# Theseus-AT/mlx-vector-db

Hardware: AMD Instinct MI355X
Metric: QPS + p50 latency, cosine top-10 batch=64: 1M×768D @1 GPU; 10M×128D @8 GPU (higher is better)
Workload: dtype f32 (int8 centred corpus x int8 query integer-MFMA candidates, fp64 exact rerank); 1 GPU; c2: 1M x 768 fp32 cosine top-10, batch 64; n_rows=1000000, dim=768, global_batch=64, batch_per_gpu_equiv=64, k=10, metric=cosine, parallelism=single GPU, rows_per_gpu=1000000

## Files before the change

### mlx-vector-db_amd/csrc/vdb_api.cpp

```cpp
#include <hip/hip_runtime.h>

#include <algorithm>
#include <atomic>
#include <cmath>
#include <cstdarg>
#include <cstdio>
#include <cstring>
#include <mutex>
#include <set>
#include <unordered_map>
#include <shared_mutex>
#include <string>
#include <vector>

#include "../../include/vdb.h"
#include "vdb_compact_plan.h"
#include "vdb_internal.h"

using namespace vdb;

namespace {

thread_local std::string g_last_error;

// ... 79 lines not shown
    float* d_dir = nullptr;
    bool dir_set = false;
    double xres_dir = 0.0;
    float* d_mu = nullptr;
    float sx = 0.0f;
    int64_t dir_rows = 0;
    unsigned long long* d_i8 = nullptr;
    double i8st[6] = {0, 0, 0, 0, 0, 0};
    uint32_t* d_csum = nullptr;
    int64_t scan_checksum = 1;
    bool auto_i8 = true;
    hipStream_t stream = nullptr;
    int n_cu = 256;
    int64_t precision = VDB_PREC_AUTO;
    std::atomic<int> auto_hold{0}, auto_fails{0}, auto_ok{0};
    std::atomic<int> auto_hold8{0}, auto_fails8{0}, auto_ok8{0};
    std::atomic<bool> last_i8{false};
    std::atomic<unsigned long long> auto_seen{0};
    unsigned long long* h_totals = nullptr;
    int64_t margin = -1;
    int64_t force_exact = 0;
    int64_t n_wg_override = 0;
    int64_t timing = 0;
    int64_t pilot_tiles = -1;
    int64_t graph_fill = 0;
    int64_t scan_variant = 0;
    int64_t scan_variant_b3 = 0;
    int64_t scan_sync = 0;
    int64_t no_fallback = 0;
    int64_t pilot_rank_override = 0;
    bool no_dir_bound = false;
    int64_t finish_split = 1;
    int64_t finish_small = -1;
    int64_t scan_qlds = -1;
    int i8_refine = -1;
    int64_t device_repass = -1;
    std::atomic<int> repass_arm{0};
    int64_t i8_narrow = -1;
    std::atomic<bool> i8_wide{false};
    std::atomic<bool> auto_i8q{true};
    std::atomic<bool> i8q_off{false};
    std::atomic<bool> last_i8q{false};
    std::atomic<int> last_i8q_b{0};
    int64_t scan_q4 = -1;
    int64_t scan_wide = -1;
    int64_t remove_chunk = 0;
    std::atomic<int64_t> gen{0};
    std::atomic<int64_t> n_searches{0}, n_queries{0}, n_fallback{0}, n_overflow{0}, n_incons{0}, n_repass{0}, n_q4{0};
    std::atomic<int64_t> n_wide{0};
    std::atomic<int64_t> n_xs_builds{0};
    std::atomic<int64_t> n_rows_removed{0};
    std::atomic<int64_t> n_by_prec[N_PREC] = {{0}, {0}, {0}, {0}, {0}, {0}};
    std::atomic<int64_t> scan_ns{0}, pipe_ns{0}, n_timed{0};
    unsigned long long* d_totals = nullptr;
    std::shared_mutex mu;
    std::mutex xs_mu;
    std::mutex ws_mu;
    std::vector<Workspace*> pool;
    std::unordered_map<hipStream_t, hipEvent_t> uses;
};

namespace {

std::mutex g_reg_mu;
std::set<vdb_index*> g_indices;

void free_workspace_memory(Workspace* w) {
    if (w->dev) (void)hipFree(w->dev);
    if (w->exact) (void)hipFree(w->exact);
    if (w->host_flag) (void)hipHostFree(w->host_flag);
    if (w->host_io) (void)hipHostFree(w->host_io);
    w->dev = nullptr;
    w->exact = nullptr;
    w->host_flag = nullptr;
    w->host_io = nullptr;
    w->dev_bytes = w->exact_bytes = w->host_io_bytes = 0;
}

int wait_idle(vdb_index* ix);

enum XsKind { kXsNone = -1, kXsFp32 = 0, kXsSplit = 1 };
int xs_kind(int64_t precision) {
// ... 536 lines not shown
        }
        if (xq && ix->X && ix->count > 0) {
            HIP_TRY(build_candidate_rows(ix, 0, ix->count, ix->stream, false, true));
            HIP_TRY(read_i8_stats(ix, ix->stream));
        }
    } else if (n == "margin") {
        ix->margin = value;
    } else if (n == "force_exact") {
        ix->force_exact = value != 0;
    } else if (n == "n_wg") {
        ix->n_wg_override = value;
    } else if (n == "scan_sync") {
        if (value < 0 || value > 2) return set_error(VDB_ERR_INVALID, "scan_sync must be 0, 1 or 2");
        ix->scan_sync = value;
    } else if (n == "scan_variant") {
        if (value < 0 || value > 2) return set_error(VDB_ERR_INVALID, "scan_variant must be 0, 1 or 2");
        ix->scan_variant = value;
    } else if (n == "scan_variant_bf16x3") {
        if (value != 0) return set_error(VDB_ERR_INVALID, "the split-bf16 pass has one variant (0)");
        ix->scan_variant_b3 = value;
    } else if (n == "graph_fill") {
        if (value < 0 || value > 1) return set_error(VDB_ERR_INVALID, "graph_fill must be 0 or 1");
        ix->graph_fill = value;
    } else if (n == "pilot_tiles") {
        if (value < -1 || value > 32768) return set_error(VDB_ERR_INVALID, "pilot_tiles must be in [-1, 32768]");
        ix->pilot_tiles = value;
    } else if (n == "timing") {
        ix->timing = value != 0;
    } else if (n == "no_fallback") {
        ix->no_fallback = value != 0;
    } else if (n == "finish_small") {
        if (value < -1 || value > 1) return set_error(VDB_ERR_INVALID, "finish_small must be -1, 0 or 1");
        ix->finish_small = value;
    } else if (n == "finish_split") {
        if (value < 1 || value > 8) return set_error(VDB_ERR_INVALID, "finish_split must be in [1, 8]");
        ix->finish_split = value;
    } else if (n == "scan_qlds") {
        if (value < -1 || value > 2) return set_error(VDB_ERR_INVALID, "scan_qlds must be -1 (auto), 0, 1 or 2");
        ix->scan_qlds = value;
    } else if (n == "scan_wide") {
        if (value < -1 || value > 1) return set_error(VDB_ERR_INVALID, "scan_wide must be -1, 0 or 1");
        ix->scan_wide = value;
    } else if (n == "scan_q4") {
        if (value < -1 || value > 1) return set_error(VDB_ERR_INVALID, "scan_q4 must be -1, 0 or 1");
        ix->scan_q4 = value;
    } else if (n == "dir_bound") {
        ix->no_dir_bound = value == 0;
    } else if (n == "i8_refine") {
        if (value < -1 || value > 1) return set_error(VDB_ERR_INVALID, "i8_refine must be -1, 0 or 1");
        ix->i8_refine = (int)value;
    } else if (n == "i8_narrow") {
        if (value < -1 || value > 0) return set_error(VDB_ERR_INVALID, "i8_narrow must be -1 or 0");
        ix->i8_narrow = value;
    } else if (n == "remove_chunk") {
        if (value < 0) return set_error(VDB_ERR_INVALID, "remove_chunk must be >= 0 (0 = sized by bytes)");
        std::unique_lock<std::shared_mutex> g(ix->mu);
        ix->remove_chunk = value;
    } else if (n == "device_repass") {
        if (value < -1 || value > 1) return set_error(VDB_ERR_INVALID, "device_repass must be -1, 0 or 1");
        ix->device_repass = value;
    } else if (n.rfind("debug_", 0) == 0 && !debug_knobs_enabled()) {
        return set_error(VDB_ERR_INVALID, "'%s' is a test-only knob (set VDB_DEBUG_KNOBS=1)", name);
    } else if (n == "debug_sink_row8") {
        HIP_TRY(hipSetDevice(ix->device));
        std::unique_lock<std::shared_mutex> g(ix->mu);
        if (value < 0 || value >= ix->count || !ix->Xq)
// ... 16 lines not shown
        HIP_TRY(hipMemcpyAsync(ix->rinit32 + value, &zero, sizeof(float), hipMemcpyHostToDevice, ix->stream));
        HIP_TRY(hipStreamSynchronize(ix->stream));
    } else if (n == "pilot_rank") {
        if (value < 0 || value > 256) return set_error(VDB_ERR_INVALID, "pilot_rank must be in [0, 256]");
        ix->pilot_rank_override = value;
    } else {
        return set_error(VDB_ERR_INVALID, "unknown parameter '%s'", name);
    }
    return VDB_OK;
}

int32_t vdb_index_get_stat(const vdb_index* cix, const char* name, int64_t* value) {
    if (!cix || !name || !value) return set_error(VDB_ERR_INVALID, "NULL argument");
    vdb_index* ix = const_cast<vdb_index*>(cix);
    std::string n(name);
    unsigned long long dt[4] = {0, 0, 0, 0};
    if ((n == "fallback_queries" || n == "overflow_queries" || n == "repass_queries") && ix->d_totals) {
        HIP_TRY(hipSetDevice(ix->device));
        const int wr = wait_idle(ix);
        if (wr) return wr;
        HIP_TRY(hipMemcpy(dt, ix->d_totals, sizeof(dt), hipMemcpyDeviceToHost));
    }
    if (n == "scan_ns" || n == "pipeline_ns" || n == "timed_searches") {
        HIP_TRY(hipSetDevice(ix->device));
        const int rc = flush_all_timing(ix);
        if (rc) return rc;
    }
    if (n == "searches") *value = ix->n_searches.load();
    else if (n == "queries") *value = ix->n_queries.load();
    else if (n == "fallback_queries") *value = ix->n_fallback.load() + (int64_t)dt[0];
    else if (n == "repass_queries") *value = ix->n_repass.load() + (int64_t)dt[3];
    else if (n == "searches_q4") *value = ix->n_q4.load();
    else if (n == "searches_wide") *value = ix->n_wide.load();
    else if (n == "auto_hold") *value = ix->auto_hold.load();
    else if (n == "auto_hold8") *value = ix->auto_hold8.load();
    else if (n == "overflow_queries") *value = ix->n_overflow.load() + (int64_t)dt[1];
    else if (n == "inconsistent_queries") *value = ix->n_incons.load();
    else if (n == "capacity") *value = ix->cap_rows;
    else if (n == "scan_ns") *value = ix->scan_ns.load();
    else if (n == "pipeline_ns") *value = ix->pipe_ns.load();
    else if (n == "timed_searches") *value = ix->n_timed.load();
    else if (n == "count") *value = ix->count;
    else if (n == "precision") *value = ix->precision;
    else if (n == "searches_fp32") *value = ix->n_by_prec[PREC_FP32].load();
    else if (n == "searches_bf16x3") *value = ix->n_by_prec[PREC_BF16X3].load();
    else if (n == "searches_bf16") *value = ix->n_by_prec[PREC_BF16].load();
    else if (n == "searches_i8") *value = ix->n_by_prec[PREC_I8].load();
    else if (n == "searches_i8x3") *value = ix->n_by_prec[PREC_I8X3].load();
    else if (n == "auto_int8") *value = ix->auto_i8 ? 1 : 0;
    else if (n == "auto_i8q") *value = ix->auto_i8q ? 1 : 0;
    else if (n == "i8q_off") *value = ix->i8q_off.load() ? 1 : 0;
    else if (n == "searches_i8q") *value = ix->n_by_prec[PREC_I8Q].load();
    else if (n == "i8_wide") *value = ix->i8_wide ? 1 : 0;
    else if (n == "device_bytes") {
        const int64_t xb = (int64_t)(ix->cap_rows / 32) * ix->G * BLOCK_FLOATS * 4;
        *value = xb + (xs_ptr(ix) ? xb : 0) + (ix->Xq ? xb / 2 : 0) + (ix->Xh ? xb / 4 : 0) + ix->cap_rows * 20;
    } else if (n == "split_copy") *value = xs_ptr(ix) ? 1 : 0;
    else if (n == "split_copy_builds") *value = ix->n_xs_builds.load();
    else if (n == "rows_removed") *value = ix->n_rows_removed.load();
    else return set_error(VDB_ERR_INVALID, "unknown stat '%s'", name);
    return VDB_OK;
}

constexpr int64_t kDirRows = 65536;

static hipError_t setup_direction(vdb_index* ix, int64_t row0, int64_t n, hipStream_t st) {
// ... 325 lines not shown
    if (!ix || (!out_host && n > 0)) return set_error(VDB_ERR_INVALID, "NULL argument");
    if (start < 0 || n < 0 || start + n > ix->count)
        return set_error(VDB_ERR_INVALID, "rows [%lld, %lld) out of range [0, %lld)", (long long)start,
                         (long long)(start + n), (long long)ix->count);
    if (n == 0) return VDB_OK;
    HIP_TRY(hipSetDevice(ix->device));
    std::shared_lock<std::shared_mutex> g(ix->mu);
    const int D = ix->dim;
    const int64_t chunk = std::max<int64_t>(1, (int64_t)(256ll << 20) / ((int64_t)D * 4));
    float* tmp = nullptr;
    HIP_TRY(hipMalloc(&tmp, (size_t)std::min(chunk, n) * D * sizeof(float)));
    for (int64_t r = 0; r < n; r += chunk) {
        const int64_t m = std::min(chunk, n - r);
        hipError_t e = launch_unpack_rows(ix->X, ix->G, D, start + r, m, tmp, ix->stream);
        if (e == hipSuccess)
            e = hipMemcpyAsync(out_host + r * D, tmp, (size_t)m * D * sizeof(float), hipMemcpyDeviceToHost, ix->stream);
        if (e == hipSuccess) e = hipStreamSynchronize(ix->stream);
        if (e != hipSuccess) {
            (void)hipFree(tmp);
            return set_error(VDB_ERR_HIP, "export failed: %s", hipGetErrorString(e));
        }
    }
    (void)hipFree(tmp);
    return VDB_OK;
}

constexpr int32_t kRetryBf16x3 = 1 << 20;
constexpr int kRepassMax = 64;
constexpr int kRepassDev = 16;
constexpr int kRepassArm = 256;
constexpr int64_t kI8NarrowRows = 512 * 1024;
constexpr int64_t kI8NarrowRowsShort = 4 * 1024 * 1024;
constexpr int64_t kWideMinRows = 65536;
constexpr int64_t kWideSplitMaxRows = 2500000;
constexpr int FIN_SEG_MAX = 512;
constexpr int64_t kRefineMinDp = 512;
constexpr int kAutoBf16MaxK = 16;

void auto_fail(vdb_index* ix) {
    const int f = std::min(8, ix->auto_fails.load() + 1);
    ix->auto_fails = f;
    ix->auto_ok = 0;
    ix->auto_hold = 16 << (f - 1);
}

bool auto_take_hold(vdb_index* ix) {
    int h = ix->auto_hold.load();
    while (h > 0)
        if (ix->auto_hold.compare_exchange_weak(h, h - 1)) return true;
    if (++ix->auto_ok >= 64) ix->auto_fails = 0;
    return false;
}

void auto_fail8(vdb_index* ix) {
    const int f = std::min(8, ix->auto_fails8.load() + 1);
    ix->auto_fails8 = f;
    ix->auto_ok8 = 0;
    ix->auto_hold8 = 16 << (f - 1);
}
bool auto_take_hold8(vdb_index* ix) {
    int h = ix->auto_hold8.load();
    while (h > 0)
        if (ix->auto_hold8.compare_exchange_weak(h, h - 1)) return true;
    if (++ix->auto_ok8 >= 64) ix->auto_fails8 = 0;
    return false;
}
// ... 242 lines not shown
    Carver c{w->dev};
    float* Qraw = c.take<float>((size_t)B * D);
    uint32_t* maskd = c.take<uint32_t>(mask_words + 64);
    float* Qt = c.take<float>((size_t)Bp * (ix->Dp + 16 * QG_EXTRA));
    double* qn64 = c.take<double>(Bp);
    double* qconst = c.take<double>((size_t)Bp * 3);
    const float* q_mu = i8_pass ? ix->d_mu : nullptr;
    const float* q_dir = (prec == PREC_BF16 || i8_pass) && ix->dir_set && !ix->no_dir_bound ? ix->d_dir : nullptr;
    float* os = c.take<float>((size_t)B * k);
    int64_t* oi = c.take<int64_t>((size_t)B * k);
    double* ok = c.take<double>((size_t)B * k);
    int* flags = c.take<int>(B + 64);
    int* done = c.take<int>(Bp);
    uint32_t* gthr = c.take<uint32_t>(Bp);
    uint32_t* gslots = c.take<uint32_t>((size_t)Bp * (KP_MAX + PILOT_SLOTS));
    uint32_t* pslots = gslots + (size_t)Bp * KP_MAX;
    float* gl_s = c.take<float>((size_t)B * gl_cap);
    uint32_t* gl_i = c.take<uint32_t>((size_t)B * gl_cap);
    uint32_t* gl_cnt = c.take<uint32_t>(Bp);
    double* fx_ek = fin_split > 1 ? c.take<double>((size_t)B * fin_split * KP_MAX) : nullptr;
    uint32_t* fx_ck = fin_split > 1 ? c.take<uint32_t>((size_t)B * fin_split * KP_MAX) : nullptr;
    uint32_t* fx_cr = fin_split > 1 ? c.take<uint32_t>((size_t)B * fin_split * KP_MAX) : nullptr;
    int* fx_n = fin_split > 1 ? c.take<int>((size_t)B * fin_split) : nullptr;
    float* q8max = c.take<float>(Bp);
    float* q8lsl = c.take<float>(Bp);
    float* q8err = c.take<float>(Bp);
    float* q8scal = c.take<float>(64);
    float* q8res = i8_refine ? c.take<float>((size_t)Bp * ix->Dp) : nullptr;
    float* q8err2 = i8_refine ? c.take<float>(Bp) : nullptr;
    uint32_t* chkp = chk ? c.take<uint32_t>((size_t)2 * n_wg8 * Bp) : nullptr;
    uint32_t* segc = wide8 ? c.take<uint32_t>((size_t)Bp * n_seg8) : nullptr;
    uint32_t* chkr = chk && ix->metric == 1 ? c.take<uint32_t>(64) : nullptr;
    int* rs8 = rs8_on ? c.take<int>((size_t)round_up(N, 32)) : nullptr;
    uint32_t* chke = chk && n_pilot > 0 ? c.take<uint32_t>((size_t)2 * Bp) : nullptr;
    float* rep_q = mem == VDB_MEM_DEVICE ? c.take<float>((size_t)R_rep * D) : nullptr;
    float* rep_s = mem == VDB_MEM_DEVICE ? c.take<float>((size_t)R_rep * k) : nullptr;
    int64_t* rep_i = mem == VDB_MEM_DEVICE ? c.take<int64_t>((size_t)R_rep * k) : nullptr;
    double* rep_k = mem == VDB_MEM_DEVICE ? c.take<double>((size_t)R_rep * k) : nullptr;

    const float* Qd = queries;
    const uint32_t* md = row_mask;
    float* out_s = out_scores;
    int64_t* out_i = out_indices;
    double* out_k = out_keys;
    const size_t io_q = mem == VDB_MEM_HOST ? (size_t)B * D * 4 : 0;
    const size_t io_r = (size_t)B * k * (4 + 8 + (out_keys ? 8 : 0));
    bool staged = false;
    if (mem == VDB_MEM_HOST) {
        rc = ws_host_io(w, io_q + io_r);
        if (rc) return rc;
        std::memcpy(w->host_io, queries, io_q);
        HIP_TRY(hipMemcpyAsync(Qraw, w->host_io, io_q, hipMemcpyHostToDevice, st));
        Qd = Qraw;
        if (row_mask && N > 0) {
            HIP_TRY(hipMemcpyAsync(maskd, row_mask, (size_t)mask_words * 4, hipMemcpyHostToDevice, st));
            md = maskd;
        }
        out_s = os;
        out_i = oi;
        out_k = out_keys ? ok : nullptr;
    }

    if (N == 0) {
        HIP_TRY(launch_empty_results((int64_t)B * k, out_s, out_i, out_k, st));
    } else {
        HIP_TRY(launch_prep_queries(Qd, B, Bp, D, ix->G, ix->metric, prec == PREC_FP32 ? Qt : nullptr,
                                    split_pass ? Qt : nullptr, qn64, flags, gthr, gslots, gl_cnt, done, st,
                                    i8_pass ? q8max : nullptr, q_mu, q_dir, qconst));
        if (i8_pass && !exact_all) {
            Int8Consts c8;
            c8.sx = ix->sx;
            c8.zmax_h = ix->i8st[4];
            c8.xl_max = ix->i8st[5];
            c8.rmax_half = 0.5 * ix->xmax * ix->xmax;
            HIP_TRY(launch_prep8(Qd, qn64, q8max, B, Bp, D, Gs, ix->metric, prec, c8, Qt, q8lsl, q8err, q8scal, st,
                                 q8res, q8err2));
            if (rs8) {
                if (chkr) HIP_TRY(hipMemsetAsync(chkr, 0, sizeof(uint32_t), st));
                HIP_TRY(launch_rstart8(ix->rinit32, N, q8scal, rs8, chkr, st));
            }
        }
        int n_flag = 0;
        if (!exact_all) {
            const bool timed = ix->timing != 0 && !opt.gate;
            hipEvent_t* tev = nullptr;
            if (timed) {
                if (w->t_pending == Workspace::kTRing) {
                    const int frc = flush_timing(ix, w, 1);
                    if (frc) return frc;
                }
                tev = w->tring[w->t_head];
                w->t_head = (w->t_head + 1) % Workspace::kTRing;
                w->t_pending++;
                for (int e = 0; e < 4; ++e)
                    if (!tev[e]) HIP_TRY(hipEventCreate(&tev[e]));
                HIP_TRY(hipEventRecord(tev[3], st));
            }
            const float* rowscale = ix->metric == 0 ? ix->inv32 : ix->sq32;
            const float* Xscan = i8_pass ? ix->Xq : xs_ptr(ix);
            if (n_pilot > 0) {
                if (i8_pass) {
                    HIP_TRY(launch_pilot8(prec, ix->metric, Xscan, ix->rinit32, md, Qt, q8scal, Gs, N, B,
                                          (B + QB_pilot - 1) / QB_pilot, QB_pilot, n_pilot, pslots, st,
                                          chke ? ix->d_csum : nullptr, chke, wide_long));
                    HIP_TRY(launch_pilot_bound(pslots, B, pilot_rank, gthr, st));
                } else if (split_pass) {
                    HIP_TRY(launch_pilot2(prec, ix->metric, pilot_rank, Xscan, ix->rinit32, md, Qt, Gs, N, B,
                                          (B + QB_pilot - 1) / QB_pilot, QB_pilot, n_pilot, pslots, gthr, st));
                    HIP_TRY(launch_pilot_bound(pslots, B, pilot_rank, gthr, st));
                }
                else
                    HIP_TRY(launch_pilot(prec, ix->metric, pilot_rank, Xscan, rowscale, md, Qt, Gs, N, B,
                                         n_qblocks, QB, n_pilot, pslots, gthr, st));
            }
            if (opt.gate && (q4 || !(split_pass || i8_pass)))
                return set_error(VDB_ERR_INVALID, "device re-pass: the sub-search has no gated candidate pass");
            if (timed) HIP_TRY(hipEventRecord(tev[0], st));
            if (q4) ix->n_q4++;
            if (wide8) ix->n_wide++;
            if (wide_long)
                HIP_TRY(launch_scan8wl(prec, ix->metric, Xscan, md, Qt, q8lsl, q8scal, Gs, N, B, n_seg8, gl_s, gl_i,
                                       gl_cap, segc, gthr, chkp, st));
            else if (wide8)
                HIP_TRY(launch_scan8w(prec, ix->metric, Xscan, rs8, md, Qt, q8lsl, q8scal, Gs, N, B, Bp, n_seg8, gl_s, gl_i,
                                      gl_cap, segc, gthr, chkp, Bp, chk_l ? 1 : 0, st));
            else if (i8_pass)
                HIP_TRY(launch_scan8(prec, ix->metric, KP, Xscan, (const float*)rs8, md, Qt, q8lsl, q8scal, Gs, N, B,
                                     n_qblocks, n_steps, n_wg, spw, gl_s, gl_i, gl_cnt, gl_cap, gthr, lockstep,
                                     (int)ix->scan_qlds, st, opt.gate, chkp, Bp, chk_l ? 1 : 0));
            else if (split_pass)
                HIP_TRY(launch_scan2(prec, ix->metric, KP, Xscan, ix->rinit32, md, Qt, Gs, N, B, n_qblocks, n_steps,
                                     n_wg, spw, gl_s, gl_i, gl_cnt, gl_cap, gthr, lockstep, st, q4,
                                     (int)ix->scan_qlds, opt.gate));
            else if (priv)
                HIP_TRY(launch_scan_topk_priv(prec, ix->metric, KP, Xscan, rowscale, md, Qt, Gs, N, B, n_qblocks,
                                              n_steps, n_wg, spw, gl_s, gl_i, gl_cnt, gl_cap, gthr, gslots, st));
            else
// ... 21 lines not shown
                fa.qerr = q8err;
                fa.mu = ix->d_mu;
                if (i8_refine) {
                    fa.xh_rm = ix->Xh;
                    fa.qres = q8res;
                    fa.qerr2 = q8err2;
                    fa.qscal = q8scal;
                    fa.sx = ix->sx;
                    fa.Dp = ix->Dp;
                }
            }
            fa.out_s = out_s; fa.out_i = out_i; fa.out_k = out_k; fa.index_offset = index_offset;
            fa.row_ids = row_ids;
            fa.flag_count = flags; fa.flag_list = flags + 1; fa.gthr = gthr; fa.overflow_count = flags + B + 1;
            fa.incons_count = flags + B + 2;
            fa.gate = opt.gate;
            if (chk) {
                fa.chkp = chkp;
                fa.chke = chke;
                fa.chkr = chkr;
                fa.chk_q = Qt;
                fa.chk_csum = ix->d_csum;
                fa.chk_g8 = Gs;
                fa.chk_nw = n_wg8;
                fa.chk_ld = Bp;
                fa.chk_l = chk_l;
            }
            fa.qconst = fa.mu == q_mu && fa.dir == q_dir ? qconst : nullptr;
            fa.seg_cnt = segc;
            fa.seg_n = n_seg8;
            fa.small = D <= 1024 && (ix->finish_small == 1 ||
                                     (ix->finish_small < 0 && B >= 32 &&
                                      ((wide_long && Gs <= 32) || (wide8 && !wide_long)) &&
                                      others_in_flight(ix, w))) ? 1 : 0;
            fa.split = fin_split; fa.sx_ek = fx_ek; fa.sx_ck = fx_ck; fa.sx_cr = fx_cr; fa.sx_n = fx_n; fa.done = done;
            HIP_TRY(launch_finish(ix->metric, KP, fa, B, st));
            if (timed) HIP_TRY(hipEventRecord(tev[2], st));
            if (ix->no_fallback && mem == VDB_MEM_DEVICE) return VDB_OK;
            if (!ix->no_fallback && mem == VDB_MEM_DEVICE && exact_bytes(ix, B, k, true) <= kGatedExactBytes) {
                {
                    std::lock_guard<std::mutex> lg(ix->ws_mu);
                    if (!ix->d_totals) {
                        HIP_TRY(hipHostMalloc(&ix->h_totals, 2 * sizeof(unsigned long long), hipHostMallocDefault));
                        ix->h_totals[0] = ix->h_totals[1] = 0;
                        unsigned long long* d = nullptr;
                        HIP_TRY(hipMalloc(&d, 4 * sizeof(unsigned long long)));
                        HIP_TRY(zero_now(d, 4 * sizeof(unsigned long long), ix->stream));
                        ix->d_totals = d;
                    }
                }
                unsigned long long* htot =
                    auto_prec && (one_plane || prec == PREC_I8X3 || prec == PREC_I8Q) ? ix->h_totals : nullptr;
                const bool can_rep = !opt.repass && auto_prec && (one_plane || prec == PREC_I8X3 || prec == PREC_I8Q) &&
                                     xs_kind(VDB_PREC_BF16X3) == xs_kind(ix->precision) && rep_q &&
                                     k <= kMaxApproxK;
                bool rep = can_rep && ix->device_repass == 1;
                if (can_rep && ix->device_repass < 0) {
                    int a = ix->repass_arm.load();
                    while (a > 0 && !ix->repass_arm.compare_exchange_weak(a, a - 1)) {}
                    rep = a > 0;
                }
                if (rep) {
                    int* counts = flags + B + 3;
                    HIP_TRY(launch_repass_gather(Qd, D, flags, R_rep, rep_q, counts, ix->d_totals + 3, st));
                    SearchOpts o;
                    o.force_b3 = true;
                    o.force_i8x3 = true;
// ... 640 lines not shown
```

### mlx-vector-db_amd/csrc/vdb_internal.h

```cpp
#pragma once
#include <hip/hip_runtime.h>
#include <stdint.h>

namespace vdb {

constexpr int TILE_ROWS = 32;
constexpr int GROUP_DIMS = 8;
constexpr int BLOCK_FLOATS = 256;
constexpr int QG_EXTRA = 8;
constexpr int ROW_ALIGN = 1024;

constexpr int PREC_FP32 = 0;
constexpr int PREC_BF16X3 = 1;
constexpr int PREC_BF16 = 2;
constexpr int PREC_I8 = 3;
constexpr int PREC_I8X3 = 4;
constexpr int PREC_I8Q = 5;
constexpr int N_PREC = 6;
inline bool prec_is_i8(int p) { return p == PREC_I8 || p == PREC_I8X3 || p == PREC_I8Q; }

struct Int8Consts {
    float sx;
    double zmax_h, xl_max, rmax_half;
};
hipError_t launch_zmax(const float* X, const float* inv32, const float* mu, int64_t row0, int64_t n, int D, int G,
                       uint32_t* out, hipStream_t st);
hipError_t launch_quant_rows(const float* X, const float* inv32, const float* mu, const float* dir, float sx,
                             int64_t row0, int64_t n, int G, float* Xq, unsigned long long* stats, hipStream_t st, int8_t* xh_rm = nullptr);
hipError_t launch_prep8(const float* Q, const double* qn64, const float* qmax, int B, int Bp, int D, int G8,
                        int metric, int prec, const Int8Consts& c, float* Qq, float* lsl, float* qerr, float* qscal,
                        hipStream_t st, float* qres = nullptr, float* qerr2 = nullptr);
hipError_t launch_colsum8(const float* Xq, int64_t row0, int64_t n, int G8, uint32_t* csum, hipStream_t st);
hipError_t launch_rstart8(const float* rinit, int64_t N, const float* qscal, int* rs, uint32_t* sum, hipStream_t st);
hipError_t launch_sink_row8(float* Xq, int64_t row, int G8, hipStream_t st);
hipError_t launch_pilot8(int prec, int metric, const float* Xq, const float* rinit, const uint32_t* mask,
                         const float* Qq, const float* qscal, int G8, int64_t N, int B, int n_qblocks, int QB,
                         int n_sample, uint32_t* pslots, hipStream_t st, const uint32_t* csum = nullptr,
                         uint32_t* chke = nullptr, bool wide = false);
int scan8_rows_per_step(int prec, int metric);
constexpr int W8_CH = 32;
bool scan8w_ok(int G8, int B);
bool scan8wl_ok(int prec, int metric, int G8, int B);
hipError_t launch_scan8wl(int prec, int metric, const float* Xq, const uint32_t* mask, const float* Qq,
                          const float* lsl, const float* qscal, int G8, int64_t N, int B, int n_seg, float* gl_s,
                          uint32_t* gl_i, int64_t gl_cap, uint32_t* seg_cnt, const uint32_t* gthr, uint32_t* chkp,
                          hipStream_t st);
hipError_t launch_scan8w(int prec, int metric, const float* Xq, const int* rs8, const uint32_t* mask, const float* Qq,
                         const float* lsl, const float* qscal, int G8, int64_t N, int B, int Bp, int n_seg,
                         float* gl_s, uint32_t* gl_i, int64_t gl_cap, uint32_t* seg_cnt, const uint32_t* gthr,
                         uint32_t* chkp, int chk_ld, int chk_l, hipStream_t st);
hipError_t launch_scan8(int prec, int metric, int KP, const float* Xq, const float* rinit, const uint32_t* mask,
                        const float* Qq, const float* lsl, const float* qscal, int G8, int64_t N, int B,
                        int n_qblocks, int64_t n_steps, int n_wg, int spw, float* gl_s, uint32_t* gl_i,
                        uint32_t* gl_cnt, int64_t gl_cap, uint32_t* gthr,
                        int lockstep, int qlds, hipStream_t st, const int* gate = nullptr,
                        uint32_t* chkp = nullptr, int chk_ld = 0, int chk_l = 0);

hipError_t launch_pack_rows(const float* src, int64_t n, int D, int G, float* X, int64_t row0,
                            double* nrm64, float* inv32, float* sq32, float* rinit32, int normalise,
                            unsigned long long* xmax_bits, int* nonfinite, hipStream_t st);

hipError_t launch_dir_sum(const float* X, const float* inv32, int64_t row0, int64_t n, int D, int G, double* sums,
                          hipStream_t st);
hipError_t launch_resid_dir(const float* X, const float* inv32, int64_t row0, int64_t n, int D, int G,
// ... 175 lines not shown
```

### mlx-vector-db_amd/csrc/vdb_scan8.hip

```cpp
#include "vdb_scan8_kernel.h"

#ifndef VDB_S8_QLDS_BIG_G8
#define VDB_S8_QLDS_BIG_G8 16
#endif

namespace vdb {

__global__ void __launch_bounds__(256) zmax_kernel(const float* __restrict__ X, const float* __restrict__ inv32,
                                                   const float* __restrict__ mu, int64_t row0, int64_t n, int D, int G,
                                                   uint32_t* __restrict__ out) {
    const int lane = threadIdx.x & 63;
    const int64_t i = (int64_t)blockIdx.x * 4 + (threadIdx.x >> 6);
    float m = 0.0f;
    if (i < n) {
        const uint64_t r = (uint64_t)(row0 + i);
        const float iv = inv32 ? inv32[r] : 1.0f;
        for (int d = lane; d < D; d += 64) {
            const float x = X[row_piece_offset(r, d >> 2, G) + (d & 3)];
            m = fmaxf(m, fabsf((inv32 ? x * iv : x) - mu[d]));
        }
    }
#pragma unroll
    for (int off = 32; off >= 1; off >>= 1) m = fmaxf(m, __shfl_xor(m, off, 64));
    if (lane == 0 && i < n) atomicMax(out, __float_as_uint(m));
// ... 250 lines not shown
            for (int j4 = 0; j4 < 4; ++j4) {
                f32x4 v;
#pragma unroll
                for (int j = 0; j < 4; ++j) {
                    const int d = d0 + 4 * j4 + j;
                    const float qv = (real && d < D) ? q[d] * scale : 0.0f;
                    v[j] = qv - sq * (float)hv[4 * j4 + j];
                }
                *(f32x4*)(rd + 4 * j4) = v;
            }
        }
    }
    s_rq = wave_sum_butterfly(s_rq);
    s_r8 = wave_sum_butterfly(s_r8);
    s_ql = wave_sum_butterfly(s_ql);
    s_qh = wave_sum_butterfly(s_qh);
    if (lane == 0) {
        const bool x3 = prec == PREC_I8X3, q16 = x3 || prec == PREC_I8Q;
        const double za = c.zmax_h + (x3 ? c.xl_max : 0.0);
        const double sl = q16 ? c.zmax_h * sqrt(s_ql) + (x3 ? c.xl_max * sqrt(s_qh) : 0.0) : 0.0;
        double e = za * sqrt(q16 ? s_rq : s_r8) + (x3 ? c.xl_max * sqrt(s_ql) : 0.0) + (metric == 1 ? (double)uH : 0.0);
        e = 1.01 * (metric == 0 ? e : 2.0 * e);
        lsl[b] = real ? (float)(1.01 * sl) * (1.0f + 1e-5f) + 1e-30f : 0.0f;
        qerr[b] = real ? (float)e * (1.0f + 1e-5f) : 0.0f;
        if (qerr2) qerr2[b] = real ? (float)(1.01 * (metric == 1 ? 2.0 * (double)uH : 0.0)) * (1.0f + 1e-5f) : 0.0f;
    }
}

hipError_t launch_prep8(const float* Q, const double* qn64, const float* qmax, int B, int Bp, int D, int G8,
                        int metric, int prec, const Int8Consts& c, float* Qq, float* lsl, float* qerr, float* qscal,
                        hipStream_t st, float* qres, float* qerr2) {
    hipLaunchKernelGGL(prep8_kernel, dim3((Bp + 3) / 4), dim3(256), 0, st, Q, qn64, qmax, B, Bp, D, G8, metric, prec, c,
                       Qq, lsl, qerr, qscal, qres, qerr2);
    return hipGetLastError();
}

constexpr int PILOT8_WAVES = 4;
#ifndef VDB_PILOT8_W1
#define VDB_PILOT8_W1 0
#endif
__host__ __device__ inline int pilot8_w(int G8, bool wide = false) {
    return VDB_PILOT8_W1 || (G8 > 24 && !wide) ? 1 : G8 >= 16 ? 4 : G8 >= 8 ? 2 : 1;
}

template <int PREC>
__device__ __forceinline__ void pilot8_chke(const float* __restrict__ Qq, int G, int B,
                                            const uint32_t* __restrict__ csum, uint32_t* __restrict__ chke) {
    constexpr size_t PLANE = 4 * BLOCK_FLOATS;
    constexpr bool HL = Planes8<PREC>::L;
    const int wv_ = threadIdx.x >> 6, ln = threadIdx.x & 63;
    const int GQ = G + QG_EXTRA, Dp = 32 * G;
    for (int q = blockIdx.x * PILOT8_WAVES + wv_; q < B; q += gridDim.x * PILOT8_WAVES) {
        uint32_t eh = 0u, el = 0u;
        for (int cc = ln; cc < 2 * G; cc += 64) {
            const int g = cc >> 1, h = cc & 1, d0 = 32 * g + 16 * h;
            const float* src = Qq + s2_blk((uint64_t)(q >> 5), g, GQ) + (size_t)((q & 31) + 32 * h) * 4;
            const f32x4 qh4 = *(const f32x4*)src;
            const f32x4 ql4 = *(const f32x4*)(src + PLANE);
#pragma unroll
            for (int w = 0; w < 4; ++w) {
                const uint32_t uh = __float_as_uint(qh4[w]), ul = __float_as_uint(ql4[w]);
#pragma unroll
                for (int bt = 0; bt < 4; ++bt) {
                    const int d = d0 + 4 * w + bt;
                    const uint32_t hv = (uint32_t)(int)(int8_t)((uh >> (8 * bt)) & 255u);
                    const uint32_t ch = csum[d];
// ... 246 lines not shown
```

Measured before the change: 483,900 queries/s.

## Fuse int8 query preparation, prep8, and checksum setup into one kernel

Adds a fused prep_i8 kernel that handles query norms, centring constants, int8 quantisation, error bounds, workspace resets and the pilot checksum in a single launch. It replaces the separate prep_queries, prep8 and memset launches plus the checksum work inside pilot8. Each workgroup redundantly computes the global max over all queries so no separate reduction pass is needed. This is meant to cut launch and serialisation overhead for small batches, at the cost of redundant per-block work over the whole batch. It is enabled automatically only when B*Dp is at most 64K floats and no other searches are in flight.

```diff
diff --git a/mlx-vector-db_amd/csrc/vdb_api.cpp b/mlx-vector-db_amd/csrc/vdb_api.cpp
--- a/mlx-vector-db_amd/csrc/vdb_api.cpp
+++ b/mlx-vector-db_amd/csrc/vdb_api.cpp
@@ -135,6 +135,7 @@
     bool no_dir_bound = false;
     int64_t finish_split = 1;
     int64_t finish_small = -1;
+    int64_t prep_fused = -1;
     int64_t scan_qlds = -1;
     int i8_refine = -1;
     int64_t device_repass = -1;
@@ -151,6 +152,7 @@
     std::atomic<int64_t> gen{0};
     std::atomic<int64_t> n_searches{0}, n_queries{0}, n_fallback{0}, n_overflow{0}, n_incons{0}, n_repass{0}, n_q4{0};
     std::atomic<int64_t> n_wide{0};
+    std::atomic<int64_t> n_prep_fused{0};
     std::atomic<int64_t> n_xs_builds{0};
     std::atomic<int64_t> n_rows_removed{0};
     std::atomic<int64_t> n_by_prec[N_PREC] = {{0}, {0}, {0}, {0}, {0}, {0}};
@@ -753,6 +755,9 @@
     } else if (n == "finish_small") {
         if (value < -1 || value > 1) return set_error(VDB_ERR_INVALID, "finish_small must be -1, 0 or 1");
         ix->finish_small = value;
+    } else if (n == "prep_fused") {
+        if (value < -1 || value > 1) return set_error(VDB_ERR_INVALID, "prep_fused must be -1, 0 or 1");
+        ix->prep_fused = value;
     } else if (n == "finish_split") {
         if (value < 1 || value > 8) return set_error(VDB_ERR_INVALID, "finish_split must be in [1, 8]");
         ix->finish_split = value;
@@ -835,6 +840,7 @@
     else if (n == "repass_queries") *value = ix->n_repass.load() + (int64_t)dt[3];
     else if (n == "searches_q4") *value = ix->n_q4.load();
     else if (n == "searches_wide") *value = ix->n_wide.load();
+    else if (n == "searches_prep_fused") *value = ix->n_prep_fused.load();
     else if (n == "auto_hold") *value = ix->auto_hold.load();
     else if (n == "auto_hold8") *value = ix->auto_hold8.load();
     else if (n == "overflow_queries") *value = ix->n_overflow.load() + (int64_t)dt[1];
@@ -1226,6 +1232,7 @@
 constexpr int64_t kI8NarrowRows = 512 * 1024;
 constexpr int64_t kI8NarrowRowsShort = 4 * 1024 * 1024;
 constexpr int64_t kWideMinRows = 65536;
+constexpr int64_t kPrepFusedMaxFloats = 65536;
 constexpr int64_t kWideSplitMaxRows = 2500000;
 constexpr int FIN_SEG_MAX = 512;
 constexpr int64_t kRefineMinDp = 512;
@@ -1534,7 +1541,15 @@
     uint32_t* segc = wide8 ? c.take<uint32_t>((size_t)Bp * n_seg8) : nullptr;
     uint32_t* chkr = chk && ix->metric == 1 ? c.take<uint32_t>(64) : nullptr;
     int* rs8 = rs8_on ? c.take<int>((size_t)round_up(N, 32)) : nullptr;
-    uint32_t* chke = chk && n_pilot > 0 ? c.take<uint32_t>((size_t)2 * Bp) : nullptr;
+    int oif = -1;
+    auto others = [&]() {
+        if (oif != 0) oif = others_in_flight(ix, w) ? 1 : 0;
+        return oif == 1;
+    };
+    const bool prep_fused = i8_pass && !exact_all && N > 0 &&
+                            (ix->prep_fused == 1 ||
+                             (ix->prep_fused < 0 && (int64_t)B * ix->Dp <= kPrepFusedMaxFloats && !others()));
+    uint32_t* chke = chk && (prep_fused || n_pilot > 0) ? c.take<uint32_t>((size_t)2 * Bp) : nullptr;
     float* rep_q = mem == VDB_MEM_DEVICE ? c.take<float>((size_t)R_rep * D) : nullptr;
     float* rep_s = mem == VDB_MEM_DEVICE ? c.take<float>((size_t)R_rep * k) : nullptr;
     int64_t* rep_i = mem == VDB_MEM_DEVICE ? c.take<int64_t>((size_t)R_rep * k) : nullptr;
@@ -1566,19 +1581,27 @@
     if (N == 0) {
         HIP_TRY(launch_empty_results((int64_t)B * k, out_s, out_i, out_k, st));
     } else {
-        HIP_TRY(launch_prep_queries(Qd, B, Bp, D, ix->G, ix->metric, prec == PREC_FP32 ? Qt : nullptr,
-                                    split_pass ? Qt : nullptr, qn64, flags, gthr, gslots, gl_cnt, done, st,
-                                    i8_pass ? q8max : nullptr, q_mu, q_dir, qconst));
+        if (!prep_fused)
+            HIP_TRY(launch_prep_queries(Qd, B, Bp, D, ix->G, ix->metric, prec == PREC_FP32 ? Qt : nullptr,
+                                        split_pass ? Qt : nullptr, qn64, flags, gthr, gslots, gl_cnt, done, st,
+                                        i8_pass ? q8max : nullptr, q_mu, q_dir, qconst));
         if (i8_pass && !exact_all) {
             Int8Consts c8;
             c8.sx = ix->sx;
             c8.zmax_h = ix->i8st[4];
             c8.xl_max = ix->i8st[5];
             c8.rmax_half = 0.5 * ix->xmax * ix->xmax;
-            HIP_TRY(launch_prep8(Qd, qn64, q8max, B, Bp, D, Gs, ix->metric, prec, c8, Qt, q8lsl, q8err, q8scal, st,
-                                 q8res, q8err2));
+            if (prep_fused) {
+                HIP_TRY(launch_prep_i8(Qd, B, Bp, D, Gs, ix->metric, prec, c8, q_mu, q_dir, qn64, qconst, q8max, flags,
+                                       gthr, gl_cnt, done, pslots, Qt, q8lsl, q8err, q8scal, q8res, q8err2,
+                                       chke ? ix->d_csum : nullptr, chke, chkr, st));
+                ix->n_prep_fused++;
+            } else {
+                HIP_TRY(launch_prep8(Qd, qn64, q8max, B, Bp, D, Gs, ix->metric, prec, c8, Qt, q8lsl, q8err, q8scal, st,
+                                     q8res, q8err2));
+            }
             if (rs8) {
-                if (chkr) HIP_TRY(hipMemsetAsync(chkr, 0, sizeof(uint32_t), st));
+                if (chkr && !prep_fused) HIP_TRY(hipMemsetAsync(chkr, 0, sizeof(uint32_t), st));
                 HIP_TRY(launch_rstart8(ix->rinit32, N, q8scal, rs8, chkr, st));
             }
         }
@@ -1604,7 +1627,8 @@
                 if (i8_pass) {
                     HIP_TRY(launch_pilot8(prec, ix->metric, Xscan, ix->rinit32, md, Qt, q8scal, Gs, N, B,
                                           (B + QB_pilot - 1) / QB_pilot, QB_pilot, n_pilot, pslots, st,
-                                          chke ? ix->d_csum : nullptr, chke, wide_long));
+                                          chke && !prep_fused ? ix->d_csum : nullptr, prep_fused ? nullptr : chke,
+                                          wide_long));
                     HIP_TRY(launch_pilot_bound(pslots, B, pilot_rank, gthr, st));
                 } else if (split_pass) {
                     HIP_TRY(launch_pilot2(prec, ix->metric, pilot_rank, Xscan, ix->rinit32, md, Qt, Gs, N, B,
@@ -1692,7 +1716,7 @@
             fa.small = D <= 1024 && (ix->finish_small == 1 ||
                                      (ix->finish_small < 0 && B >= 32 &&
                                       ((wide_long && Gs <= 32) || (wide8 && !wide_long)) &&
-                                      others_in_flight(ix, w))) ? 1 : 0;
+                                      others())) ? 1 : 0;
             fa.split = fin_split; fa.sx_ek = fx_ek; fa.sx_ck = fx_ck; fa.sx_cr = fx_cr; fa.sx_n = fx_n; fa.done = done;
             HIP_TRY(launch_finish(ix->metric, KP, fa, B, st));
             if (timed) HIP_TRY(hipEventRecord(tev[2], st));
diff --git a/mlx-vector-db_amd/csrc/vdb_internal.h b/mlx-vector-db_amd/csrc/vdb_internal.h
--- a/mlx-vector-db_amd/csrc/vdb_internal.h
+++ b/mlx-vector-db_amd/csrc/vdb_internal.h
@@ -30,6 +30,11 @@
 hipError_t launch_prep8(const float* Q, const double* qn64, const float* qmax, int B, int Bp, int D, int G8,
                         int metric, int prec, const Int8Consts& c, float* Qq, float* lsl, float* qerr, float* qscal,
                         hipStream_t st, float* qres = nullptr, float* qerr2 = nullptr);
+hipError_t launch_prep_i8(const float* Q, int B, int Bp, int D, int G8, int metric, int prec, const Int8Consts& c,
+                          const float* mu, const float* dir, double* qn64, double* qconst, float* qmax,
+                          int* flag_count, uint32_t* gthr, uint32_t* gl_cnt, int* done, uint32_t* pslots, float* Qq,
+                          float* lsl, float* qerr, float* qscal, float* qres, float* qerr2, const uint32_t* csum,
+                          uint32_t* chke, uint32_t* chkr, hipStream_t st);
 hipError_t launch_colsum8(const float* Xq, int64_t row0, int64_t n, int G8, uint32_t* csum, hipStream_t st);
 hipError_t launch_rstart8(const float* rinit, int64_t N, const float* qscal, int* rs, uint32_t* sum, hipStream_t st);
 hipError_t launch_sink_row8(float* Xq, int64_t row, int G8, hipStream_t st);
diff --git a/mlx-vector-db_amd/csrc/vdb_scan8.hip b/mlx-vector-db_amd/csrc/vdb_scan8.hip
--- a/mlx-vector-db_amd/csrc/vdb_scan8.hip
+++ b/mlx-vector-db_amd/csrc/vdb_scan8.hip
@@ -306,6 +306,335 @@
                         hipStream_t st, float* qres, float* qerr2) {
     hipLaunchKernelGGL(prep8_kernel, dim3((Bp + 3) / 4), dim3(256), 0, st, Q, qn64, qmax, B, Bp, D, G8, metric, prec, c,
                        Qq, lsl, qerr, qscal, qres, qerr2);
+    return hipGetLastError();
+}
+
+constexpr int PREP_I8_U = 16;
+constexpr size_t PREP_I8_LDS_MAX = 48 * 1024;
+
+template <bool LDS, bool VEC>
+__global__ void __launch_bounds__(256)
+prep_i8_kernel(const float* __restrict__ Q, int B, int Bp, int D, int G8, int metric, int prec, Int8Consts c,
+               const float* __restrict__ mu, const float* __restrict__ dir, double* __restrict__ qn64,
+               double* __restrict__ qconst, float* __restrict__ qmax, int* __restrict__ flag_count,
+               uint32_t* __restrict__ gthr, uint32_t* __restrict__ gl_cnt, int* __restrict__ done,
+               uint32_t* __restrict__ pslots, float* __restrict__ Qq, float* __restrict__ lsl,
+               float* __restrict__ qerr, float* __restrict__ qscal, float* __restrict__ qres,
+               float* __restrict__ qerr2, const uint32_t* __restrict__ csum, uint32_t* __restrict__ chke,
+               uint32_t* __restrict__ chkr) {
+    extern __shared__ float s_rows[];
+    __shared__ float s_wmax[4];
+    const int lane = threadIdx.x & 63, wv = threadIdx.x >> 6;
+    const int b = blockIdx.x * 4 + wv;
+    const int Dp = 32 * G8;
+    const int np = (D + 255) / 256;
+    const bool slot = b < Bp, real = b < B;
+    const bool wg_real = blockIdx.x * 4 < B;
+    const float* q = Q + (int64_t)(real ? b : 0) * D;
+    float* s_row = s_rows + (size_t)wv * Dp;
+    float* s_mu = s_rows + (size_t)4 * Dp;
+    float* s_dir = s_rows + (size_t)5 * Dp;
+    uint32_t* s_cs = (uint32_t*)(s_rows + (size_t)6 * Dp);
+    auto load4 = [&](const float* row, bool live, int d0) {
+        f32x4 v = {0.f, 0.f, 0.f, 0.f};
+        if (live && d0 < D) {
+            if (VEC) v = *(const f32x4*)(row + d0);
+            else {
+#pragma unroll
+                for (int j = 0; j < 4; ++j) v[j] = d0 + j < D ? row[d0 + j] : 0.0f;
+            }
+        }
+        return v;
+    };
+    auto load_round = [&](f32x4 (&v)[PREP_I8_U], int j0, int m) {
+#pragma unroll
+        for (int u = 0; u < PREP_I8_U; ++u) {
+            const int j = j0 + 4 * u;
+            v[u] = load4(Q + (int64_t)(j < B ? j : 0) * D, j < B, 4 * (m * 64 + lane));
+        }
+    };
+    if (b == 0 && lane == 0) {
+        if (flag_count) {
+            flag_count[0] = 0;
+            flag_count[B + 1] = 0;
+            flag_count[B + 2] = 0;
+        }
+        if (chkr) *chkr = 0u;
+    }
+    if (slot) {
+        if (lane == 0 && gthr) gthr[b] = 0u;
+        if (lane == 0 && gl_cnt) gl_cnt[b] = 0u;
+        if (lane == 0 && done) done[b] = 0;
+        if (pslots)
+            for (int j = lane; j < PILOT_SLOTS; j += 64) pslots[pslot_at(b, j, B)] = 0u;
+    }
+    float lmax = 0.0f, am_own = 0.0f;
+    double nq = 0.0;
+    f32x4 va[PREP_I8_U], vb[PREP_I8_U];
+    if (wg_real) {
+        if (LDS) {
+            for (int base = 0; base < Dp; base += 1024) {
+                f32x4 r[4];
+#pragma unroll
+                for (int i = 0; i < 4; ++i) r[i] = load4(q, real, base + 256 * i + 4 * lane);
+                const int dc = base + 4 * (int)threadIdx.x;
+                f32x4 m4 = {0.f, 0.f, 0.f, 0.f}, d4 = {0.f, 0.f, 0.f, 0.f};
+                i32x4 ch = {0, 0, 0, 0}, cl = {0, 0, 0, 0};
+                if (dc < Dp) {
+                    if (mu) m4 = *(const f32x4*)(mu + dc);
+                    if (dir) d4 = *(const f32x4*)(dir + dc);
+                    if (chke) {
+                        ch = *(const i32x4*)(csum + dc);
+                        cl = *(const i32x4*)(csum + Dp + dc);
+                    }
+                }
+                if (base == 0) load_round(va, wv, 0);
+#pragma unroll
+                for (int i = 0; i < 4; ++i)
+                    if (base + 256 * i + 4 * lane < Dp) *(f32x4*)(s_row + base + 256 * i + 4 * lane) = r[i];
+                if (dc < Dp) {
+                    *(f32x4*)(s_mu + dc) = m4;
+                    *(f32x4*)(s_dir + dc) = d4;
+                    *(i32x4*)(s_cs + dc) = ch;
+                    *(i32x4*)(s_cs + Dp + dc) = cl;
+                }
+            }
+        } else {
+            load_round(va, wv, 0);
+        }
+    }
+    for (int j0 = wv; j0 < B && wg_real; j0 += 4 * PREP_I8_U) {
+        double acc[PREP_I8_U];
+        float am[PREP_I8_U];
+#pragma unroll
+        for (int u = 0; u < PREP_I8_U; ++u) {
+            acc[u] = 0.0;
+            am[u] = 0.0f;
+        }
+        auto take = [&](const f32x4 (&v)[PREP_I8_U]) {
+#pragma unroll
+            for (int u = 0; u < PREP_I8_U; ++u)
+#pragma unroll
+                for (int e = 0; e < 4; ++e) {
+                    const double x = (double)v[u][e];
+                    acc[u] = acc[u] + x * x;
+                    am[u] = fmaxf(am[u], fabsf(v[u][e]));
+                }
+        };
+        if (j0 != wv) load_round(va, j0, 0);
+        for (int m = 0; m < np; m += 2) {
+            load_round(vb, j0, m + 1);
+            take(va);
+            load_round(va, j0, m + 2);
+            take(vb);
+        }
+#pragma unroll
+        for (int s = 0; s < 4; ++s) {
+            const int off = 32 >> s, half = PREP_I8_U >> (s + 1);
+            const bool hi = (lane & off) != 0;
+#pragma unroll
+            for (int i = 0; i < half; ++i) {
+                const double keep = hi ? acc[i + half] : acc[i], send = hi ? acc[i] : acc[i + half];
+                acc[i] = keep + __shfl_xor(send, off, 64);
+                const float keepm = hi ? am[i + half] : am[i], sendm = hi ? am[i] : am[i + half];
+                am[i] = fmaxf(keepm, __shfl_xor(sendm, off, 64));
+            }
+        }
+#pragma unroll
+        for (int off = 2; off >= 1; off >>= 1) {
+            acc[0] = acc[0] + __shfl_xor(acc[0], off, 64);
+            am[0] = fmaxf(am[0], __shfl_xor(am[0], off, 64));
+        }
+        const double n = sqrt(acc[0]);
+        const float sc = metric == 0 ? (float)(1.0 / fmax(n, 1e-8)) : 1.0f;
+        lmax = fmaxf(lmax, am[0] * sc);
+        const int uo = (b - j0) >> 2;
+        const int src = (uo & 8 ? 32 : 0) | (uo & 4 ? 16 : 0) | (uo & 2 ? 8 : 0) | (uo & 1 ? 4 : 0);
+        const double n_o = __shfl(n, src, 64);
+        const float am_o = __shfl(am[0], src, 64);
+        if (b >= j0 && uo < PREP_I8_U) {
+            nq = n_o;
+            am_own = am_o;
+        }
+    }
+#pragma unroll
+    for (int off = 32; off >= 1; off >>= 1) lmax = fmaxf(lmax, __shfl_xor(lmax, off, 64));
+    if (lane == 0) s_wmax[wv] = lmax;
+    __syncthreads();
+    if (!slot) return;
+    if (!real) {
+        const f32x4 z = {0.f, 0.f, 0.f, 0.f};
+        const int GQ = G8 + QG_EXTRA;
+        for (int cc = lane; cc < 2 * GQ; cc += 64) {
+            const int g = cc >> 1, h = cc & 1;
+            float* dst = Qq + s2_blk((uint64_t)(b >> 5), g, GQ) + (size_t)((b & 31) + 32 * h) * 4;
+            *(f32x4*)dst = z;
+            *(f32x4*)(dst + 4 * BLOCK_FLOATS) = z;
+        }
+        if (qres)
+            for (int d0 = 4 * lane; d0 < Dp; d0 += 256) *(f32x4*)(qres + (size_t)b * (size_t)Dp + d0) = z;
+        if (lane == 0) {
+            qn64[b] = 0.0;
+            qconst[3 * (size_t)b] = qconst[3 * (size_t)b + 1] = qconst[3 * (size_t)b + 2] = 0.0;
+            lsl[b] = qerr[b] = 0.0f;
+            if (qerr2) qerr2[b] = 0.0f;
+        }
+        return;
+    }
+    const float mx = fmaxf(fmaxf(s_wmax[0], s_wmax[1]), fmaxf(s_wmax[2], s_wmax[3]));
+    float sq = mx > 0.0f ? mx / 127.0f : 1.0f;
+    if (metric == 1) sq = fmaxf(sq, (float)(c.rmax_half / ((double)c.sx * 1.0e9)));
+    const float uH = c.sx * sq;
+    if (b == 0 && lane == 0) {
+        qscal[0] = uH;
+        qscal[1] = uH * (1.0f / 256.0f);
+        qscal[2] = 1.0f / uH;
+    }
+    if (lane == 0) qn64[b] = nq;
+    const float scale = metric == 0 ? (float)(1.0 / fmax(nq, 1e-8)) : 1.0f;
+    if (lane == 0) qmax[b] = fmaxf(am_own * scale, 0.0f);
+    auto row4 = [&](int d0) {
+        if (LDS) return d0 < Dp ? *(const f32x4*)(s_row + d0) : f32x4{0.f, 0.f, 0.f, 0.f};
+        return load4(q, real, d0);
+    };
+    {
+        const double qs = metric == 0 ? 1.0 / fmax(nq, 1e-8) : 1.0;
+        double mq = 0.0, cd = 0.0, q2 = 0.0, d2 = 0.0;
+        for (int m = 0; m < np; ++m) {
+            const int d0 = 4 * (m * 64 + lane);
+            f32x4 qv = {0.f, 0.f, 0.f, 0.f}, mv = {0.f, 0.f, 0.f, 0.f}, dv = {0.f, 0.f, 0.f, 0.f};
+            if (d0 < Dp) {
+                qv = row4(d0);
+                if (LDS) {
+                    mv = *(const f32x4*)(s_mu + d0);
+                    dv = *(const f32x4*)(s_dir + d0);
+                } else {
+                    if (mu) mv = *(const f32x4*)(mu + d0);
+                    if (dir) dv = *(const f32x4*)(dir + d0);
+                }
+            }
+#pragma unroll
+            for (int j = 0; j < 4; ++j) {
+                const double x = (double)qv[j] * qs;
+                mq += x * (double)mv[j];
+                cd += x * (double)dv[j];
+                q2 += x * x;
+                d2 += (double)dv[j] * (double)dv[j];
+            }
+        }
+        mq = wave_sum_butterfly(mq);
+        cd = wave_sum_butterfly(cd);
+        q2 = wave_sum_butterfly(q2);
+        d2 = wave_sum_butterfly(d2);
+        if (lane == 0) {
+            qconst[3 * (size_t)b] = mu ? mq : 0.0;
+            qconst[3 * (size_t)b + 1] = dir ? cd : 0.0;
+            qconst[3 * (size_t)b + 2] = dir ? fmax(q2 - 2.0 * cd * cd + cd * cd * d2, 0.0) : 0.0;
+        }
+    }
+    const bool x3 = prec == PREC_I8X3, q16 = x3 || prec == PREC_I8Q;
+    const float isq = 1.0f / sq;
+    const int GQ = G8 + QG_EXTRA;
+    double s_rq = 0.0, s_r8 = 0.0, s_ql = 0.0, s_qh = 0.0;
+    uint32_t eh = 0u, el = 0u;
+    for (int cc = lane; cc < 2 * GQ; cc += 64) {
+        const int g = cc >> 1, h = cc & 1;
+        const int d0 = 32 * (g % G8) + 16 * h;
+        float qv[16];
+        int hv[16], lv[16];
+#pragma unroll
+        for (int j4 = 0; j4 < 4; ++j4) {
+            const f32x4 r = row4(d0 + 4 * j4);
+#pragma unroll
+            for (int j = 0; j < 4; ++j) qv[4 * j4 + j] = r[j] * scale;
+        }
+#pragma unroll
+        for (int j = 0; j < 16; ++j) {
+            split_i8(qv[j] * isq, hv[j], lv[j]);
+            if (g < G8) {
+                const double qh = (double)sq * hv[j], ql = (double)sq * lv[j] / 256.0;
+                const double r8 = (double)qv[j] - qh, rq = r8 - ql;
+                s_rq += rq * rq;
+                s_r8 += r8 * r8;
+                s_ql += ql * ql;
+                s_qh += qh * qh;
+            }
+        }
+        float* dst = Qq + s2_blk((uint64_t)(b >> 5), g, GQ) + (size_t)((b & 31) + 32 * h) * 4;
+        *(f32x4*)dst = pack_i8x16(hv);
+        *(f32x4*)(dst + 4 * BLOCK_FLOATS) = pack_i8x16(lv);
+        if (qres && g < G8) {
+            float* rd = qres + (size_t)b * (size_t)Dp + d0;
+#pragma unroll
+            for (int j4 = 0; j4 < 4; ++j4) {
+                f32x4 v;
+#pragma unroll
+                for (int j = 0; j < 4; ++j) v[j] = qv[4 * j4 + j] - sq * (float)hv[4 * j4 + j];
+                *(f32x4*)(rd + 4 * j4) = v;
+            }
+        }
+        if (chke && g < G8) {
+#pragma unroll
+            for (int j4 = 0; j4 < 4; ++j4) {
+                const uint32_t* cs = LDS ? s_cs : csum;
+                const i32x4 ch = *(const i32x4*)(cs + d0 + 4 * j4);
+                i32x4 cl = {0, 0, 0, 0};
+                if (x3) cl = *(const i32x4*)(cs + Dp + d0 + 4 * j4);
+#pragma unroll
+                for (int j = 0; j < 4; ++j) {
+                    const uint32_t hq = (uint32_t)hv[4 * j4 + j];
+                    eh += hq * (uint32_t)ch[j];
+                    if (q16) el += (uint32_t)lv[4 * j4 + j] * (uint32_t)ch[j] + hq * (uint32_t)cl[j];
+                }
+            }
+        }
+    }
+    s_rq = wave_sum_butterfly(s_rq);
+    s_r8 = wave_sum_butterfly(s_r8);
+    s_ql = wave_sum_butterfly(s_ql);
+    s_qh = wave_sum_butterfly(s_qh);
+    if (chke) {
+#pragma unroll
+        for (int off = 32; off >= 1; off >>= 1) {
+            eh += (uint32_t)__shfl_xor((int)eh, off, 64);
+            el += (uint32_t)__shfl_xor((int)el, off, 64);
+        }
+        if (lane == 0 && real) {
+            chke[2 * (size_t)b] = eh;
+            chke[2 * (size_t)b + 1] = el;
+        }
+    }
+    if (lane == 0) {
+        const double za = c.zmax_h + (x3 ? c.xl_max : 0.0);
+        const double sl = q16 ? c.zmax_h * sqrt(s_ql) + (x3 ? c.xl_max * sqrt(s_qh) : 0.0) : 0.0;
+        double e = za * sqrt(q16 ? s_rq : s_r8) + (x3 ? c.xl_max * sqrt(s_ql) : 0.0) + (metric == 1 ? (double)uH : 0.0);
+        e = 1.01 * (metric == 0 ? e : 2.0 * e);
+        lsl[b] = real ? (float)(1.01 * sl) * (1.0f + 1e-5f) + 1e-30f : 0.0f;
+        qerr[b] = real ? (float)e * (1.0f + 1e-5f) : 0.0f;
+        if (qerr2) qerr2[b] = real ? (float)(1.01 * (metric == 1 ? 2.0 * (double)uH : 0.0)) * (1.0f + 1e-5f) : 0.0f;
+    }
+}
+
+hipError_t launch_prep_i8(const float* Q, int B, int Bp, int D, int G8, int metric, int prec, const Int8Consts& c,
+                          const float* mu, const float* dir, double* qn64, double* qconst, float* qmax,
+                          int* flag_count, uint32_t* gthr, uint32_t* gl_cnt, int* done, uint32_t* pslots, float* Qq,
+                          float* lsl, float* qerr, float* qscal, float* qres, float* qerr2, const uint32_t* csum,
+                          uint32_t* chke, uint32_t* chkr, hipStream_t st) {
+    if (chke && !csum) return hipErrorInvalidValue;
+    const size_t lds = (size_t)8 * 32 * G8 * sizeof(float);
+    const bool vec = (D & 3) == 0 && ((uintptr_t)Q & 15) == 0;
+#define VDB_PREP_I8(L, V)                                                                                        \
+    hipLaunchKernelGGL((prep_i8_kernel<L, V>), dim3((Bp + 3) / 4), dim3(256), L ? lds : 0, st, Q, B, Bp, D, G8, \
+                       metric, prec, c, mu, dir, qn64, qconst, qmax, flag_count, gthr, gl_cnt, done, pslots, Qq, \
+                       lsl, qerr, qscal, qres, qerr2, csum, chke, chkr)
+    if (lds <= PREP_I8_LDS_MAX) {
+        if (vec) VDB_PREP_I8(true, true);
+        else VDB_PREP_I8(true, false);
+    } else {
+        if (vec) VDB_PREP_I8(false, true);
+        else VDB_PREP_I8(false, false);
+    }
+#undef VDB_PREP_I8
     return hipGetLastError();
 }
 
```

Measured after the change: 482,700 queries/s. No clear change (-0.2%).
